# shaderko/velocity-asr

Hardware: NVIDIA B200
Metric: rtfx (higher is better)
Workload: dtype f32

## Files before the change

### velocity-asr_b200/csrc/scan.cu

```cuda
#include <cstdlib>
#include <map>
#include <mutex>
#include <utility>

#include "common.cuh"
#include "kernels.cuh"

namespace vasr {

namespace {

constexpr int SPL = 8;
constexpr int SCAN_THREADS = 128;
constexpr int NLEV = 26;
constexpr float LOG2E = 1.4426950408889634f;

struct State8 {
  u64 v[4];
};

__device__ __forceinline__ void powers_structured(float s, float n0p1, State8& p) {
  const float r1 = ex2_approx(s);
  const float e1 = ex2_approx(s * n0p1);
  const float r2 = r1 * r1;
// ... 477 lines not shown
  float Dv[RPL];
#pragma unroll
  for (int r = 0; r < RPL; ++r) Dv[r] = a.D ? __ldg(a.D + d0 + rl0 + r) : 0.f;

  u64 H[RPL][8];
#pragma unroll
  for (int r = 0; r < RPL; ++r)
#pragma unroll
    for (int k = 0; k < 8; ++k) H[r][k] = 0ull;

  const float* gB = a.Bm + b * L * a.ldb;
  const float* gC = a.Cm + b * L * a.ldc;
  const float* gX = a.x + b * L * a.ldx + d0;
  const float* gDt = a.dt + b * L * a.lddt + d0;
  const float* gZ = gate ? a.z + b * L * a.ldz + d0 : nullptr;
  float* gY = a.y + b * L * a.ldy + d0 + rl0;

  auto issue = [&](int c) {
    const int st = c % 3;
    const int64_t tc0 = (int64_t)c * TCH;
    const int tcn = c >= nchunks ? 0 : (int)((L - tc0) < TCH ? (L - tc0) : TCH);
    float* dB = sB(st); float* dC = sC(st); float* dX = sX(st); float* dD = sDt(st); float* dZ = sZ(st);
#pragma unroll
    for (int i = 0; i < (TCH * NF + THREADS - 1) / THREADS; ++i) {
      const int idx = tid + i * THREADS;
      const int t = idx / NF, f = idx % NF;
      if (idx < TCH * NF && t < tcn) {
        cp_async16(dB + t * N + 4 * f, gB + (tc0 + t) * a.ldb + 4 * f);
        cp_async16(dC + t * N + 4 * f, gC + (tc0 + t) * a.ldc + 4 * f);
      }
    }
#pragma unroll
    for (int i = 0; i < (TCH * RF + THREADS - 1) / THREADS; ++i) {
      const int idx = tid + i * THREADS;
      const int t = idx / RF, f = idx % RF;
      if (idx < TCH * RF && t < tcn) {
        cp_async16(dX + t * ROWS + 4 * f, gX + (tc0 + t) * a.ldx + 4 * f);
        cp_async16(dD + t * ROWS + 4 * f, gDt + (tc0 + t) * a.lddt + 4 * f);
        if (gate) cp_async16(dZ + t * ROWS + 4 * f, gZ + (tc0 + t) * a.ldz + 4 * f);
      }
    }
    cp_async_commit();
  };

  auto row_step = [&](u64 (&Hr)[8], float dtv, float xv, const ulonglong2 (&bq)[4], const ulonglong2 (&cq)[4]) {
    const float u = xv * dtv;
    const u64 uu = pack2(u, u);
    u64 Pa, Pb, rq2 = 0ull;
    if (STRUCT) {
      const float r = ex2_approx(dtv * c_r);
      const float e = ex2_approx(dtv * c_e);
      const float rq = ex2_approx(dtv * c_q);
      const float r2 = r * r;
      Pa = pack2(e, e * r);
      Pb = mul2(Pa, pack2(r2, r2));
      rq2 = pack2(rq, rq);
    }
    u64 acc0 = 0ull, acc1 = 0ull;
#pragma unroll
    for (int m = 0; m < 4; ++m) {
      if (!STRUCT) {
        Pa = pack2(ex2_approx(dtv * al2[4 * m]), ex2_approx(dtv * al2[4 * m + 1]));
        Pb = pack2(ex2_approx(dtv * al2[4 * m + 2]), ex2_approx(dtv * al2[4 * m + 3]));
      }
      Hr[2 * m] = fma2(Pa, Hr[2 * m], mul2(uu, bq[m].x));
      Hr[2 * m + 1] = fma2(Pb, Hr[2 * m + 1], mul2(uu, bq[m].y));
      if (m == 0) {
        acc0 = mul2(Hr[0], cq[0].x);
        acc1 = mul2(Hr[1], cq[0].y);
      } else {
        acc0 = fma2(Hr[2 * m], cq[m].x, acc0);
        acc1 = fma2(Hr[2 * m + 1], cq[m].y, acc1);
      }
      if (STRUCT && m < 3) {
        Pa = mul2(Pa, rq2);
        Pb = mul2(Pb, rq2);
      }
    }
    return hsum2(add2(acc0, acc1));
  };

  struct Pre {
    u64 Pa[RPL], Pb[RPL], rq2[RPL];
    float s[RPL];
  };
  auto row_step_pre = [&](u64 (&Hr)[8], u64 Pa, u64 Pb, u64 rq2, float sc, const ulonglong2 (&bq)[4],
                          const ulonglong2 (&cq)[4]) {
    u64 acc0 = 0ull, acc1 = 0ull;
#pragma unroll
    for (int m = 0; m < 4; ++m) {
      Hr[2 * m] = fma2(Pa, Hr[2 * m], bq[m].x);
      Hr[2 * m + 1] = fma2(Pb, Hr[2 * m + 1], bq[m].y);
      if (m == 0) {
        acc0 = mul2(Hr[0], cq[0].x);
        acc1 = mul2(Hr[1], cq[0].y);
      } else {
        acc0 = fma2(Hr[2 * m], cq[m].x, acc0);
        acc1 = fma2(Hr[2 * m + 1], cq[m].y, acc1);
      }
      if (m < 3) {
        Pa = mul2(Pa, rq2);
        Pb = mul2(Pb, rq2);
      }
    }
    return sc * hsum2(add2(acc0, acc1));
  };
  float s_carry[RPL];
#pragma unroll
  for (int q = 0; q < RPL; ++q) s_carry[q] = 1.0f;

  struct Ops {
    ulonglong2 bq[4], cq[4];
    float dt[RPL], x[RPL];
  };
  auto load_ops = [&](Ops& o, const float* pB, const float* pC, const float* pX, const float* pD, int t) {
#pragma unroll
    for (int m = 0; m < 4; ++m) {
      o.bq[m] = *reinterpret_cast<const ulonglong2*>(pB + t * N + 4 * LPR * m);
      o.cq[m] = *reinterpret_cast<const ulonglong2*>(pC + t * N + 4 * LPR * m);
    }
    if (RPL == 2) {
      const float2 d2 = *reinterpret_cast<const float2*>(pD + t * ROWS);
      const float2 x2 = *reinterpret_cast<const float2*>(pX + t * ROWS);
      o.dt[0] = d2.x; o.dt[RPL - 1] = d2.y; o.x[0] = x2.x; o.x[RPL - 1] = x2.y;
    } else {
#pragma unroll
      for (int r = 0; r < RPL; ++r) { o.dt[r] = pD[t * ROWS + r]; o.x[r] = pX[t * ROWS + r]; }
    }
  };

  constexpr int SPB = TPL / RPL;
  float ypv[NV], fx[TPL], fz[TPL];
#pragma unroll
  for (int i = 0; i < NV; ++i) ypv[i] = 0.f;
#pragma unroll
  for (int i = 0; i < TPL; ++i) fx[i] = fz[i] = 0.f;
  float* fy = gY;
  int fvalid = 0;
  auto finalize = [&]() {
#pragma unroll
    for (int r = 0; r < NR; ++r) {
      const int lane_bit = LPR >> (r + 1);
      const int cnt = (NV / 2) >> r;
      const bool hi = (j & lane_bit) != 0;
#pragma unroll
      for (int i = 0; i < cnt; ++i) {
        const float mine = hi ? ypv[i + cnt] : ypv[i];
        const float other = hi ? ypv[i] : ypv[i + cnt];
        ypv[i] = mine + __shfl_xor_sync(0xffffffffu, other, lane_bit);
      }
    }
#pragma unroll
    for (int sp = 0; sp < SPB; ++sp) {
      float y[RPL];
#pragma unroll
      for (int r = 0; r < RPL; ++r) {
        y[r] = fmaf(fx[sp * RPL + r], Dv[r], ypv[sp * RPL + r]);
        if (gate) {
          const float zv = fz[sp * RPL + r];
          float sg;
          asm("rcp.approx.ftz.f32 %0, %1;" : "=f"(sg) : "f"(1.0f + ex2_approx(-zv * LOG2E)));
          y[r] *= zv * sg;
        }
      }
      if (sp < fvalid) {
        if (RPL == 2) {
          *reinterpret_cast<float2*>(fy + sp * a.ldy) = make_float2(y[0], y[RPL - 1]);
        } else {
#pragma unroll
          for (int r = 0; r < RPL; ++r) fy[sp * a.ldy + r] = y[r];
        }
      }
    }
  };

  constexpr int NST = 3;
  issue(0);
  issue(1);
  for (int c = 0; c < nchunks; ++c) {
    const int st = c % NST;
    const int64_t tc0 = (int64_t)c * TCH;
    const int tcn = (int)((L - tc0) < TCH ? (L - tc0) : TCH);
    cp_async_wait<1>();
    __syncthreads();
    issue(c + 2);
    const float* pB = sB(st) + 4 * j;
    const float* pC = sC(st) + 4 * j;
    const float* pX = sX(st) + rl0;
    const float* pD = sDt(st) + rl0;
    const float* pZ = sZ(st) + rl0;

    Ops cur;
    load_ops(cur, pB, pC, pX, pD, 0);
    Pre pre;
    auto mufu_phase = [&](const Ops& o, float (&r)[RPL], float (&e)[RPL], float (&rq)[RPL]) {
#pragma unroll
      for (int q = 0; q < RPL; ++q) {
        r[q] = ex2_approx(o.dt[q] * c_r);
        e[q] = ex2_approx(o.dt[q] * c_e);
        rq[q] = ex2_approx(o.dt[q] * c_q);
      }
    };
    auto pack_phase = [&](const Ops& o, const float (&r)[RPL], const float (&e)[RPL], const float (&rq)[RPL],
                          const float (&s_prev)[RPL], Pre& p) {
#pragma unroll
      for (int q = 0; q < RPL; ++q) {
        float u = o.x[q] * o.dt[q];
        if (fabsf(u) < 1e-12f) u = copysignf(1e-12f, u);
        float inv;
        asm("rcp.approx.ftz.f32 %0, %1;" : "=f"(inv) : "f"(u));
        const float er = e[q] * (s_prev[q] * inv);
        const float r2 = r[q] * r[q];
        p.Pa[q] = pack2(er, er * r[q]);
        p.Pb[q] = mul2(p.Pa[q], pack2(r2, r2));
        p.rq2[q] = pack2(rq[q], rq[q]);
        p.s[q] = u;
      }
    };
    if (STRUCT) {
      float r[RPL], e[RPL], rq[RPL];
      mufu_phase(cur, r, e, rq);
      pack_phase(cur, r, e, rq, s_carry, pre);
    }
#pragma unroll 4
    for (int g4 = 0; g4 < TCH; g4 += 4) {
      if (g4 >= tcn) break;
      float yp[NV];
#pragma unroll
      for (int i = 0; i < 4; ++i) {
        const int t = g4 + i;
        Ops nxt;
        load_ops(nxt, pB, pC, pX, pD, t + 1 < TCH ? t + 1 : TCH - 1);
        if (STRUCT) {
          float r[RPL], e[RPL], rq[RPL];
          Pre npre;
          yp[RPL * i] = row_step_pre(H[0], pre.Pa[0], pre.Pb[0], pre.rq2[0], pre.s[0], cur.bq, cur.cq);
          mufu_phase(nxt, r, e, rq);
#pragma unroll
          for (int q = 1; q < RPL; ++q)
            yp[RPL * i + q] = row_step_pre(H[q], pre.Pa[q], pre.Pb[q], pre.rq2[q], pre.s[q], cur.bq, cur.cq);
#pragma unroll
          for (int q = 0; q < RPL; ++q) s_carry[q] = pre.s[q];
          pack_phase(nxt, r, e, rq, s_carry, npre);
          pre = npre;
        } else {
#pragma unroll
          for (int r = 0; r < RPL; ++r) yp[RPL * i + r] = row_step(H[r], cur.dt[r], cur.x[r], cur.bq, cur.cq);
        }
        cur = nxt;
      }
      float nfx[TPL], nfz[TPL];
      const int s0 = g4 + j * SPB;
#pragma unroll
      for (int sp = 0; sp < SPB; ++sp) {
        if (RPL == 2) {
          const float2 x2 = *reinterpret_cast<const float2*>(pX + (s0 + sp) * ROWS);
          const float2 z2 = gate ? *reinterpret_cast<const float2*>(pZ + (s0 + sp) * ROWS) : make_float2(0.f, 0.f);
          nfx[sp * RPL] = x2.x; nfx[sp * RPL + RPL - 1] = x2.y;
          nfz[sp * RPL] = z2.x; nfz[sp * RPL + RPL - 1] = z2.y;
        } else {
#pragma unroll
          for (int r = 0; r < RPL; ++r) {
            nfx[sp * RPL + r] = pX[(s0 + sp) * ROWS + r];
            nfz[sp * RPL + r] = gate ? pZ[(s0 + sp) * ROWS + r] : 0.f;
          }
        }
      }
      finalize();
#pragma unroll
      for (int i = 0; i < NV; ++i) ypv[i] = yp[i];
#pragma unroll
      for (int i = 0; i < TPL; ++i) { fx[i] = nfx[i]; fz[i] = nfz[i]; }
      fy = gY + (tc0 + s0) * a.ldy;
      fvalid = tcn - s0;
    }
  }
  pdl_trigger();
  finalize();
}

struct SplitArgs {
  u64* state = nullptr;
  unsigned int* flags = nullptr;
  unsigned int epoch = 0;
  int n_slots = 0;
};

__device__ __forceinline__ u64 shfl_xor2(u64 v, int m) { return __shfl_xor_sync(0xffffffffu, v, m); }
__device__ __forceinline__ u64 bcast2(float v) { return pack2(v, v); }
__device__ __forceinline__ float rcp_approx(float x) {
  float y;
  asm("rcp.approx.ftz.f32 %0, %1;" : "=f"(y) : "f"(x));
  return y;
}
__device__ __forceinline__ unsigned long long global_ns() {
  unsigned long long t;
  asm volatile("mov.u64 %0, %%globaltimer;" : "=l"(t));
  return t;
}

template <int RP, int WARPS, int OCC>
__global__ void __launch_bounds__(WARPS * 32, OCC) scan_rp_kernel(ScanArgs a, SplitArgs sa) {
  pdl_wait();
  constexpr int N = 64, G = 8, R = 2 * RP;
  constexpr int ROWS = WARPS * G * R;
  constexpr int THREADS = WARPS * 32;
  constexpr int LDR = ROWS + 8;
  constexpr int NF = N / 4, RF = ROWS / 4;
  constexpr int STAGE_FLOATS = TCH * (2 * N + 3 * LDR);
  constexpr int NST = 3;
  constexpr int NV = 4 * RP;
  constexpr int SW = RP * 17;

  extern __shared__ __align__(16) float scan_smem[];
  auto sB = [&](int st) { return scan_smem + st * STAGE_FLOATS; };
  auto sC = [&](int st) { return scan_smem + st * STAGE_FLOATS + TCH * N; };
  auto sX = [&](int st) { return scan_smem + st * STAGE_FLOATS + 2 * TCH * N; };
  auto sDt = [&](int st) { return scan_smem + st * STAGE_FLOATS + 2 * TCH * N + TCH * LDR; };
  auto sZ = [&](int st) { return scan_smem + st * STAGE_FLOATS + 2 * TCH * N + 2 * TCH * LDR; };

  const int tid = threadIdx.x;
  const int lane = tid & 31, warp = tid >> 5;
  const int g = lane >> 2, j = lane & 3;
  const int rl0 = (warp * G + g) * R;
  const int64_t L = a.L;
  const bool gate = a.z != nullptr;
  const int tiles = a.Di / ROWS;
  const int64_t cpc = (L + TCH - 1) / TCH;
  const int64_t n_chains = a.B * tiles;

  int64_t f0, f1;
  if (sa.n_slots > 0) {
    const int64_t total = n_chains * cpc;
    f0 = total * blockIdx.x / sa.n_slots;
    f1 = total * (blockIdx.x + 1) / sa.n_slots;
  } else {
    f0 = (int64_t)blockIdx.x * cpc;
    f1 = f0 + cpc;
  }
  if (f1 <= f0) {
    pdl_trigger();
    return;
  }
  const int64_t c_first = f0 / cpc, c_last = (f1 - 1) / cpc;

  const u64 CR = bcast2(-LOG2E);
  const u64 CE = bcast2(-LOG2E * (float)(4 * j + 1));
  const u64 CQ = bcast2(-LOG2E * 16.0f);

  for (int64_t chain = c_last; chain >= c_first; --chain) {
    const int cb = (int)((f0 > chain * cpc ? f0 : chain * cpc) - chain * cpc);
    const int ce = (int)((f1 < (chain + 1) * cpc ? f1 : (chain + 1) * cpc) - chain * cpc);
    const bool load_state = cb > 0, save_state = ce < cpc;
    const bool last_piece = chain == c_first;
    const int64_t b = chain / tiles;
    const int d0 = (int)(chain % tiles) * ROWS;

    u64 DV[RP];
#pragma unroll
    for (int p = 0; p < RP; ++p)
      DV[p] = a.D ? pack2(__ldg(a.D + d0 + rl0 + 2 * p), __ldg(a.D + d0 + rl0 + 2 * p + 1)) : 0ull;

    const float* gB = a.Bm + b * L * a.ldb;
    const float* gC = a.Cm + b * L * a.ldc;
    const float* gX = a.x + b * L * a.ldx + d0;
    const float* gDt = a.dt + b * L * a.lddt + d0;
    const float* gZ = gate ? a.z + b * L * a.ldz + d0 : nullptr;
    float* gY = a.y + b * L * a.ldy + d0 + rl0;

    constexpr int TSB = THREADS / NF, TSX = THREADS / RF;
    static_assert(THREADS % NF == 0 && THREADS % RF == 0 && TCH % TSB == 0 && TCH % TSX == 0, "tile shape");
    const int tb = tid / NF, fb = tid % NF, tx = tid / RF, fx = tid % RF;
    const float* qB = gB + ((int64_t)cb * TCH + tb) * a.ldb + 4 * fb;
    const float* qC = gC + ((int64_t)cb * TCH + tb) * a.ldc + 4 * fb;
    const float* qX = gX + ((int64_t)cb * TCH + tx) * a.ldx + 4 * fx;
    const float* qD = gDt + ((int64_t)cb * TCH + tx) * a.lddt + 4 * fx;
    const float* qZ = gate ? gZ + ((int64_t)cb * TCH + tx) * a.ldz + 4 * fx : nullptr;
    const int oB = tb * N + 4 * fb, oX = tx * LDR + 4 * fx;
    int c_issue = cb;
    auto issue = [&]() {
      const int c = c_issue++;
      if (c < ce) {
        const int st = (c - cb) % NST;
        float* dB = sB(st) + oB; float* dC = sC(st) + oB;
        float* dX = sX(st) + oX; float* dD = sDt(st) + oX; float* dZ = sZ(st) + oX;
        const int64_t left = L - (int64_t)c * TCH;
        if (left >= TCH) {
#pragma unroll
          for (int i = 0; i < TCH / TSB; ++i) {
            cp_async16(dB + i * TSB * N, qB + (int64_t)i * TSB * a.ldb);
            cp_async16(dC + i * TSB * N, qC + (int64_t)i * TSB * a.ldc);
          }
#pragma unroll
          for (int i = 0; i < TCH / TSX; ++i) {
            cp_async16(dX + i * TSX * LDR, qX + (int64_t)i * TSX * a.ldx);
            cp_async16(dD + i * TSX * LDR, qD + (int64_t)i * TSX * a.lddt);
            if (gate) cp_async16(dZ + i * TSX * LDR, qZ + (int64_t)i * TSX * a.ldz);
          }
        } else {
#pragma unroll
          for (int i = 0; i < TCH / TSB; ++i)
            if (tb + i * TSB < left) {
              cp_async16(dB + i * TSB * N, qB + (int64_t)i * TSB * a.ldb);
              cp_async16(dC + i * TSB * N, qC + (int64_t)i * TSB * a.ldc);
            }
#pragma unroll
          for (int i = 0; i < TCH / TSX; ++i)
            if (tx + i * TSX < left) {
              cp_async16(dX + i * TSX * LDR, qX + (int64_t)i * TSX * a.ldx);
              cp_async16(dD + i * TSX * LDR, qD + (int64_t)i * TSX * a.lddt);
              if (gate) cp_async16(dZ + i * TSX * LDR, qZ + (int64_t)i * TSX * a.ldz);
            }
        }
        qB += (int64_t)TCH * a.ldb; qC += (int64_t)TCH * a.ldc;
        qX += (int64_t)TCH * a.ldx; qD += (int64_t)TCH * a.lddt;
        if (gate) qZ += (int64_t)TCH * a.ldz;
      }
      cp_async_commit();
    };
#pragma unroll
    for (int i = 0; i < NST - 1; ++i) issue();

    u64 H[RP][16];
    u64 s_carry[RP];
    if (load_state) {
      if (tid == 0) {
        const volatile unsigned int* fl = sa.flags + (blockIdx.x - 1);
        const unsigned long long t0 = global_ns();
        while (*fl != sa.epoch) {
          __nanosleep(100);
          if (global_ns() - t0 > 4000000000ull) __trap();
        }
        __threadfence();
      }
      __syncthreads();
      const u64* st = sa.state + (size_t)(blockIdx.x - 1) * THREADS * SW + tid;
#pragma unroll
      for (int p = 0; p < RP; ++p) {
#pragma unroll
        for (int k = 0; k < 16; ++k) H[p][k] = __ldcg(st + (size_t)(p * 16 + k) * THREADS);
        s_carry[p] = __ldcg(st + (size_t)(RP * 16 + p) * THREADS);
      }
    } else {
#pragma unroll
      for (int p = 0; p < RP; ++p) {
#pragma unroll
        for (int k = 0; k < 16; ++k) H[p][k] = 0ull;
        s_carry[p] = bcast2(1.0f);
      }
    }

    struct Pre {
      u64 ER[RP], R1[RP], R2[RP], RQ[RP], S[RP];
    };
    struct Raw {
      float r[R], e[R], q[R], u[R], inv[R];
    };
    auto load_dx = [&](u64 (&DT)[RP], u64 (&X)[RP], const float* pD, const float* pX, int t) {
      if (RP == 2) {
        const ulonglong2 d = *reinterpret_cast<const ulonglong2*>(pD + t * LDR);
        const ulonglong2 x = *reinterpret_cast<const ulonglong2*>(pX + t * LDR);
        DT[0] = d.x; DT[RP - 1] = d.y; X[0] = x.x; X[RP - 1] = x.y;
      } else {
        DT[0] = *reinterpret_cast<const u64*>(pD + t * LDR);
        X[0] = *reinterpret_cast<const u64*>(pX + t * LDR);
      }
    };
    auto mufu_phase = [&](const u64 (&DT)[RP], const u64 (&X)[RP], Raw& w) {
#pragma unroll
      for (int p = 0; p < RP; ++p) {
        float a0, a1;
        unpack2(mul2(DT[p], CR), a0, a1);
        w.r[2 * p] = ex2_approx(a0); w.r[2 * p + 1] = ex2_approx(a1);
        unpack2(mul2(DT[p], CE), a0, a1);
        w.e[2 * p] = ex2_approx(a0); w.e[2 * p + 1] = ex2_approx(a1);
        unpack2(mul2(DT[p], CQ), a0, a1);
        w.q[2 * p] = ex2_approx(a0); w.q[2 * p + 1] = ex2_approx(a1);
        unpack2(mul2(X[p], DT[p]), a0, a1);
        if (fabsf(a0) < 1e-12f) a0 = copysignf(1e-12f, a0);
        if (fabsf(a1) < 1e-12f) a1 = copysignf(1e-12f, a1);
        w.u[2 * p] = a0; w.u[2 * p + 1] = a1;
        w.inv[2 * p] = rcp_approx(a0); w.inv[2 * p + 1] = rcp_approx(a1);
      }
    };
    auto pack_phase = [&](const Raw& w, const u64 (&s_prev)[RP], Pre& o) {
#pragma unroll
      for (int p = 0; p < RP; ++p) {
        const u64 ratio = mul2(s_prev[p], pack2(w.inv[2 * p], w.inv[2 * p + 1]));
        o.ER[p] = mul2(pack2(w.e[2 * p], w.e[2 * p + 1]), ratio);
        o.R1[p] = pack2(w.r[2 * p], w.r[2 * p + 1]);
        o.R2[p] = mul2(o.R1[p], o.R1[p]);
        o.RQ[p] = pack2(w.q[2 * p], w.q[2 * p + 1]);
        o.S[p] = pack2(w.u[2 * p], w.u[2 * p + 1]);
      }
    };

    u64 ypv[NV], FX[RP], FZ[RP];
#pragma unroll
    for (int i = 0; i < NV; ++i) ypv[i] = 0ull;
#pragma unroll
    for (int p = 0; p < RP; ++p) FX[p] = FZ[p] = 0ull;
    float* fy = gY;
    bool fvalid = false;
    auto finalize = [&]() {
#pragma unroll
      for (int r = 0; r < 2; ++r) {
        const int lane_bit = 2 >> r;
        const int cnt = (NV / 2) >> r;
        const bool hi = (j & lane_bit) != 0;
#pragma unroll
        for (int i = 0; i < cnt; ++i) {
          const u64 mine = hi ? ypv[i + cnt] : ypv[i];
          const u64 other = hi ? ypv[i] : ypv[i + cnt];
          ypv[i] = add2(mine, shfl_xor2(other, lane_bit));
        }
      }
      float out[R];
#pragma unroll
      for (int p = 0; p < RP; ++p) {
        u64 y = fma2(FX[p], DV[p], ypv[p]);
        if (gate) {
          float e0, e1;
          unpack2(mul2(FZ[p], CR), e0, e1);
          const u64 sg = pack2(rcp_approx(1.0f + ex2_approx(e0)), rcp_approx(1.0f + ex2_approx(e1)));
          y = mul2(y, mul2(FZ[p], sg));
        }
        unpack2(y, out[2 * p], out[2 * p + 1]);
      }
      if (fvalid) {
        if (RP == 2) *reinterpret_cast<float4*>(fy) = make_float4(out[0], out[1], out[R - 2], out[R - 1]);
        else *reinterpret_cast<float2*>(fy) = make_float2(out[0], out[1]);
      }
    };

    cp_async_wait<NST - 2>();
    __syncthreads();
    Pre pre;
    {
      u64 DT[RP], X[RP];
      Raw w;
      load_dx(DT, X, sDt(0) + rl0, sX(0) + rl0, 0);
      mufu_phase(DT, X, w);
      pack_phase(w, s_carry, pre);
    }
    for (int c = cb; c < ce; ++c) {
      const int st = (c - cb) % NST, stn = (c + 1 - cb) % NST;
      const int64_t tc0 = (int64_t)c * TCH;
      const int tcn = (int)((L - tc0) < TCH ? (L - tc0) : TCH);
      if (last_piece && c + 1 == ce) pdl_trigger();
      const float* pB = sB(st) + 4 * j;
      const float* pC = sC(st) + 4 * j;
      const float* pX = sX(st) + rl0;
      const float* pD = sDt(st) + rl0;
      const float* pZ = sZ(st) + rl0;
#pragma unroll 1
      for (int g4 = 0; g4 < TCH; g4 += 4) {
        if (g4 >= tcn) break;
        const bool last_block = g4 + 4 == TCH;
        if (last_block) {
          cp_async_wait<0>();
          __syncthreads();
          issue();
        }
        const float* pDl = last_block ? sDt(stn) + rl0 : pD + (g4 + 4) * LDR;
        const float* pXl = last_block ? sX(stn) + rl0 : pX + (g4 + 4) * LDR;
        u64 yp[NV];
#pragma unroll
        for (int i = 0; i < 4; ++i) {
          const int t = g4 + i;
          u64 DTn[RP], Xn[RP];
          Raw w;
          Pre npre;
          if (i < 3) load_dx(DTn, Xn, pD, pX, t + 1);
          else load_dx(DTn, Xn, pDl, pXl, 0);
          u64 P[RP][4], acc[RP][2];
#pragma unroll
          for (int p = 0; p < RP; ++p) {
            P[p][0] = pre.ER[p];
            P[p][1] = mul2(pre.ER[p], pre.R1[p]);
            P[p][2] = mul2(pre.ER[p], pre.R2[p]);
            P[p][3] = mul2(P[p][1], pre.R2[p]);
          }
#pragma unroll
          for (int m = 0; m < 4; ++m) {
            const float4 bq = *reinterpret_cast<const float4*>(pB + t * N + 16 * m);
            const float4 cq = *reinterpret_cast<const float4*>(pC + t * N + 16 * m);
            const float bv[4] = {bq.x, bq.y, bq.z, bq.w};
            const float cv[4] = {cq.x, cq.y, cq.z, cq.w};
#pragma unroll
            for (int p = 0; p < RP; ++p) {
#pragma unroll
              for (int q = 0; q < 4; ++q) {
                u64& h = H[p][4 * m + q];
                h = fma2(P[p][q], h, bcast2(bv[q]));
                if (m == 0 && q < 2) acc[p][q] = mul2(h, bcast2(cv[q]));
                else acc[p][q & 1] = fma2(h, bcast2(cv[q]), acc[p][q & 1]);
                if (m < 3) P[p][q] = mul2(P[p][q], pre.RQ[p]);
              }
            }
            if (m == 0) mufu_phase(DTn, Xn, w);
          }
#pragma unroll
          for (int p = 0; p < RP; ++p) {
            yp[RP * i + p] = mul2(add2(acc[p][0], acc[p][1]), pre.S[p]);
            s_carry[p] = pre.S[p];
          }
          pack_phase(w, s_carry, npre);
          pre = npre;
        }
        u64 nFX[RP], nFZ[RP];
        const int s0 = g4 + j;
        if (RP == 2) {
          const ulonglong2 x2 = *reinterpret_cast<const ulonglong2*>(pX + s0 * LDR);
          nFX[0] = x2.x; nFX[RP - 1] = x2.y;
          if (gate) {
            const ulonglong2 z2 = *reinterpret_cast<const ulonglong2*>(pZ + s0 * LDR);
            nFZ[0] = z2.x; nFZ[RP - 1] = z2.y;
          } else {
            nFZ[0] = nFZ[RP - 1] = 0ull;
          }
        } else {
          nFX[0] = *reinterpret_cast<const u64*>(pX + s0 * LDR);
          nFZ[0] = gate ? *reinterpret_cast<const u64*>(pZ + s0 * LDR) : 0ull;
        }
        finalize();
#pragma unroll
        for (int i = 0; i < NV; ++i) ypv[i] = yp[i];
#pragma unroll
        for (int p = 0; p < RP; ++p) { FX[p] = nFX[p]; FZ[p] = nFZ[p]; }
        fy = gY + (tc0 + s0) * a.ldy;
        fvalid = s0 < tcn;
      }
    }
    finalize();
    cp_async_wait<0>();

    if (save_state) {
      u64* st = sa.state + (size_t)blockIdx.x * THREADS * SW + tid;
#pragma unroll
      for (int p = 0; p < RP; ++p) {
#pragma unroll
        for (int k = 0; k < 16; ++k) __stcg(st + (size_t)(p * 16 + k) * THREADS, H[p][k]);
        __stcg(st + (size_t)(RP * 16 + p) * THREADS, s_carry[p]);
      }
      __threadfence();
      __syncthreads();
      if (tid == 0) *reinterpret_cast<volatile unsigned int*>(sa.flags + blockIdx.x) = sa.epoch;
    } else {
      __syncthreads();
    }
  }
}

constexpr int RP_WARPS = 4;
template <int RP, int OCC = 3>
struct RpCfg {
  static constexpr int ROWS = RP_WARPS * 8 * 2 * RP;
  static constexpr int THREADS = RP_WARPS * 32;
  static constexpr size_t SMEM = (size_t)3 * TCH * (2 * 64 + 3 * (ROWS + 8)) * sizeof(float);
  static constexpr size_t STATE_BYTES = (size_t)THREADS * RP * 17 * sizeof(unsigned long long);
};
constexpr int RP_MAX_SLOTS = 1024;
constexpr size_t RP_SCRATCH_BYTES = 4096 + (size_t)RP_MAX_SLOTS * RpCfg<2>::STATE_BYTES;

struct RpScratch {
  void* mem = nullptr;
  unsigned int epoch = 0;
};
cudaError_t rp_scratch(cudaStream_t s, RpScratch** out) {
  static std::mutex mu;
  static std::map<std::pair<int, cudaStream_t>, RpScratch> cache;
  int dev = 0;
  cudaError_t e = cudaGetDevice(&dev);
  if (e != cudaSuccess) return e;
  std::lock_guard<std::mutex> lock(mu);
  RpScratch& sc = cache[std::make_pair(dev, s)];
  if (!sc.mem) {
    e = cudaMalloc(&sc.mem, RP_SCRATCH_BYTES);
    if (e != cudaSuccess) return e;
    e = cudaMemset(sc.mem, 0, 4096);
    if (e != cudaSuccess) return e;
  }
  *out = &sc;
  return cudaSuccess;
}

bool rp_takes(const ScanArgs& a) {
  auto al16 = [](const void* p) { return (reinterpret_cast<uintptr_t>(p) & 15) == 0; };
  if (a.parallel_quirk || !a.structured_a || a.N != 64 || a.Di % RpCfg<1>::ROWS != 0) return false;
  if ((a.ldx & 3) || (a.lddt & 3) || (a.ldy & 3) || (a.ldb & 3) || (a.ldc & 3)) return false;
  if (!al16(a.x) || !al16(a.dt) || !al16(a.y) || !al16(a.Bm) || !al16(a.Cm)) return false;
  if (a.z && ((a.ldz & 3) || !al16(a.z))) return false;
  return true;
}

template <int RP, int OCC>
cudaError_t launch_rp_cfg(const ScanArgs& a, int sms, cudaStream_t s) {
  using C = RpCfg<RP, OCC>;
  auto kernel = scan_rp_kernel<RP, RP_WARPS, OCC>;
  constexpr size_t SPLIT_SMEM = C::SMEM > 78 * 1024 ? C::SMEM : 78 * 1024;
  static int occ = -1;
  cudaError_t e = cudaSuccess;
  if (occ < 0) {
    e = cudaFuncSetAttribute(kernel, cudaFuncAttributeMaxDynamicSharedMemorySize, (int)SPLIT_SMEM);
    if (e != cudaSuccess) return e;
    int n = 0;
    e = cudaOccupancyMaxActiveBlocksPerMultiprocessor(&n, kernel, C::THREADS, C::SMEM);
    if (e != cudaSuccess) return e;
    occ = n;
  }
  const int64_t n_chains = a.B * (a.Di / C::ROWS);
  const int64_t total = n_chains * ((a.L + TCH - 1) / TCH);
  SplitArgs sa;
  unsigned grid = (unsigned)n_chains;
  size_t smem = C::SMEM;
  int64_t slots = (int64_t)(occ < 2 ? occ : 2) * sms;
  if (slots > RP_MAX_SLOTS) slots = RP_MAX_SLOTS;
  if (slots > total) slots = total;
  static const int split_env = debug_env_int("VASR_SCAN_SPLIT", -1);
  if (split_env > 0 && split_env <= (int64_t)occ * sms && split_env <= RP_MAX_SLOTS) slots = split_env;
  bool split = occ > 0 && n_chains > slots && slots >= 1 && n_chains % slots != 0;
  if (split_env == 0) split = false;
  if (split) {
    RpScratch* sc = nullptr;
    e = rp_scratch(s, &sc);
    if (e != cudaSuccess) return e;
    sa.n_slots = (int)slots;
    sa.flags = reinterpret_cast<unsigned int*>(sc->mem);
    sa.state = reinterpret_cast<u64*>(reinterpret_cast<char*>(sc->mem) + 4096);
    if (++sc->epoch == 0) ++sc->epoch;
    sa.epoch = sc->epoch;
    grid = (unsigned)slots;
    smem = SPLIT_SMEM;
  }
  return launch_k(kernel, dim3(grid), dim3(C::THREADS), smem, s, a, sa);
}

cudaError_t launch_rp(const ScanArgs& a, cudaStream_t s) {
  const int sms = a.num_sms > 0 ? a.num_sms : 148;
  static const int rp_env = debug_env_int("VASR_SCAN_RP", 0);
  const bool wide = rp_env ? rp_env == 2 : a.B * (a.Di / RpCfg<2>::ROWS) >= 2 * sms;
  if (a.Di % RpCfg<2>::ROWS == 0 && wide) {
    return launch_rp_cfg<2, 2>(a, sms, s);
  }
  return launch_rp_cfg<1, 3>(a, sms, s);
}

template <int LPR, int WARPS, int RPL>
cudaError_t launch_seq(const ScanArgs& a, cudaStream_t s) {
  constexpr int N = LPR * 16;
  constexpr int ROWS = WARPS * (32 / LPR) * RPL;
  constexpr size_t SMEM = (size_t)3 * TCH * (2 * N + 3 * ROWS) * sizeof(float);
  dim3 grid((unsigned)(a.Di / ROWS), (unsigned)a.B);
  cudaError_t e = cudaSuccess;
  auto go = [&](auto kernel) {
    if (SMEM > 48 * 1024) e = cudaFuncSetAttribute(kernel, cudaFuncAttributeMaxDynamicSharedMemorySize, (int)SMEM);
    if (e == cudaSuccess) e = launch_k(kernel, grid, dim3(WARPS * 32), SMEM, s, a);
  };
  if (a.structured_a) go(scan_seq_kernel<LPR, WARPS, RPL, true>);
  else go(scan_seq_kernel<LPR, WARPS, RPL, false>);
  return e;
}

template <int LPR>
cudaError_t launch_recurrence(const ScanArgs& a, cudaStream_t s) {
  constexpr int G = 32 / LPR;
  auto al16 = [](const void* p) { return (reinterpret_cast<uintptr_t>(p) & 15) == 0; };
  if ((a.ldx & 3) || (a.lddt & 3) || (a.ldy & 1) || !al16(a.x) || !al16(a.dt) || (a.z && ((a.ldz & 3) || !al16(a.z))) ||
      (reinterpret_cast<uintptr_t>(a.y) & 7))
    return cudaErrorInvalidValue;
  if (4 * G * 2 <= 128 && a.Di % (4 * G * 2) == 0) return launch_seq<LPR, 4, 2>(a, s);
  if (2 * G * 2 <= 128 && a.Di % (2 * G * 2) == 0) return launch_seq<LPR, 2, 2>(a, s);
  if (a.Di % (G * 2) == 0) return launch_seq<LPR, 1, 2>(a, s);
  return cudaErrorInvalidValue;
}

template <int LPR8>
cudaError_t launch_lpr(const ScanArgs& a, cudaStream_t s) {
  if (!a.parallel_quirk) return launch_recurrence<LPR8 / 2>(a, s);
  constexpr int ROWS = SCAN_THREADS / LPR8;
  if (a.Di % ROWS != 0) return cudaErrorInvalidValue;
  dim3 grid((unsigned)(a.Di / ROWS), (unsigned)a.B);
  if (a.structured_a) return launch_k(scan_quirk_kernel<LPR8, true>, grid, dim3(SCAN_THREADS), 0, s, a);
  return launch_k(scan_quirk_kernel<LPR8, false>, grid, dim3(SCAN_THREADS), 0, s, a);
}

}

cudaError_t launch_selective_scan(const ScanArgs& a, cudaStream_t s, int64_t* launches) {
  if (a.B <= 0 || a.L <= 0) return cudaSuccess;
  if (a.B > 65535 || a.L >= (1LL << (NLEV - 2))) return cudaErrorInvalidValue;
  if ((a.ldb & 3) || (a.ldc & 3) || (reinterpret_cast<uintptr_t>(a.Bm) & 15) ||
      (reinterpret_cast<uintptr_t>(a.Cm) & 15))
    return cudaErrorInvalidValue;
  cudaError_t e;
  static const int old_env = debug_env_int("VASR_SCAN_OLD", 0);
  if (rp_takes(a) && !old_env) {
    e = launch_rp(a, s);
    if (launches && e == cudaSuccess) ++*launches;
    return e;
  }
  switch (a.N) {
    case 64: e = launch_lpr<8>(a, s); break;
    case 32: e = launch_lpr<4>(a, s); break;
    case 16: e = launch_lpr<2>(a, s); break;
    default: return cudaErrorInvalidValue;
  }
  if (launches && e == cudaSuccess) ++*launches;
  return e;
}

}
```

Baseline: 192,000.

## Precompute per-row scan seeds in shared memory and halve state per lane

Adds a per-chunk prep pass that computes decay exponentials, the ratio of consecutive u values and u itself once per row, storing them in a double-buffered shared seed area. The main loop then loads these instead of redoing the MUFU exp and reciprocal work per lane. Lanes are regrouped to 8 per row group, so each lane carries 8 state pairs instead of 16, and the s_carry rescaling moves into finalize. The RP=1 path is dropped. This adds shared memory and a prep step inside the pipeline, and the extra smem may lower occupancy.

```diff
diff --git a/velocity-asr_b200/csrc/scan.cu b/velocity-asr_b200/csrc/scan.cu
--- a/velocity-asr_b200/csrc/scan.cu
+++ b/velocity-asr_b200/csrc/scan.cu
@@ -803,7 +803,8 @@
 template <int RP, int WARPS, int OCC>
 __global__ void __launch_bounds__(WARPS * 32, OCC) scan_rp_kernel(ScanArgs a, SplitArgs sa) {
   pdl_wait();
-  constexpr int N = 64, G = 8, R = 2 * RP;
+  static_assert(RP == 2, "row pairs per lane: the seed pre-pass covers a warp's rows with two lanes per row");
+  constexpr int N = 64, G = 4, R = 2 * RP;
   constexpr int ROWS = WARPS * G * R;
   constexpr int THREADS = WARPS * 32;
   constexpr int LDR = ROWS + 8;
@@ -811,7 +812,10 @@
   constexpr int STAGE_FLOATS = TCH * (2 * N + 3 * LDR);
   constexpr int NST = 3;
   constexpr int NV = 4 * RP;
-  constexpr int SW = RP * 17;
+  constexpr int FP = RP / 2;
+  constexpr int SW = RP * 8;
+  constexpr int WR = G * R;
+  static_assert(32 % WR == 0 && 32 / WR == 2, "prep: two lanes per row, half a chunk each");
 
   extern __shared__ __align__(16) float scan_smem[];
   auto sB = [&](int st) { return scan_smem + st * STAGE_FLOATS; };
@@ -819,11 +823,13 @@
   auto sX = [&](int st) { return scan_smem + st * STAGE_FLOATS + 2 * TCH * N; };
   auto sDt = [&](int st) { return scan_smem + st * STAGE_FLOATS + 2 * TCH * N + TCH * LDR; };
   auto sZ = [&](int st) { return scan_smem + st * STAGE_FLOATS + 2 * TCH * N + 2 * TCH * LDR; };
+  auto sSeed = [&](int buf) { return scan_smem + NST * STAGE_FLOATS + buf * 4 * TCH * ROWS; };
 
   const int tid = threadIdx.x;
   const int lane = tid & 31, warp = tid >> 5;
-  const int g = lane >> 2, j = lane & 3;
+  const int g = lane >> 3, j = lane & 7;
   const int rl0 = (warp * G + g) * R;
+  const int rf0 = rl0 + 2 * FP * (j & 1);
   const int64_t L = a.L;
   const bool gate = a.z != nullptr;
   const int tiles = a.Di / ROWS;
@@ -847,7 +853,6 @@
 
   const u64 CR = bcast2(-LOG2E);
   const u64 CE = bcast2(-LOG2E * (float)(4 * j + 1));
-  const u64 CQ = bcast2(-LOG2E * 16.0f);
 
   for (int64_t chain = c_last; chain >= c_first; --chain) {
     const int cb = (int)((f0 > chain * cpc ? f0 : chain * cpc) - chain * cpc);
@@ -857,17 +862,17 @@
     const int64_t b = chain / tiles;
     const int d0 = (int)(chain % tiles) * ROWS;
 
-    u64 DV[RP];
-#pragma unroll
-    for (int p = 0; p < RP; ++p)
-      DV[p] = a.D ? pack2(__ldg(a.D + d0 + rl0 + 2 * p), __ldg(a.D + d0 + rl0 + 2 * p + 1)) : 0ull;
+    u64 DV[FP];
+#pragma unroll
+    for (int p = 0; p < FP; ++p)
+      DV[p] = a.D ? pack2(__ldg(a.D + d0 + rf0 + 2 * p), __ldg(a.D + d0 + rf0 + 2 * p + 1)) : 0ull;
 
     const float* gB = a.Bm + b * L * a.ldb;
     const float* gC = a.Cm + b * L * a.ldc;
     const float* gX = a.x + b * L * a.ldx + d0;
     const float* gDt = a.dt + b * L * a.lddt + d0;
     const float* gZ = gate ? a.z + b * L * a.ldz + d0 : nullptr;
-    float* gY = a.y + b * L * a.ldy + d0 + rl0;
+    float* gY = a.y + b * L * a.ldy + d0 + rf0;
 
     constexpr int TSB = THREADS / NF, TSX = THREADS / RF;
     static_assert(THREADS % NF == 0 && THREADS % RF == 0 && TCH % TSB == 0 && TCH % TSX == 0, "tile shape");
@@ -922,8 +927,7 @@
 #pragma unroll
     for (int i = 0; i < NST - 1; ++i) issue();
 
-    u64 H[RP][16];
-    u64 s_carry[RP];
+    u64 H[RP][8];
     if (load_state) {
       if (tid == 0) {
         const volatile unsigned int* fl = sa.flags + (blockIdx.x - 1);
@@ -937,76 +941,78 @@
       __syncthreads();
       const u64* st = sa.state + (size_t)(blockIdx.x - 1) * THREADS * SW + tid;
 #pragma unroll
-      for (int p = 0; p < RP; ++p) {
-#pragma unroll
-        for (int k = 0; k < 16; ++k) H[p][k] = __ldcg(st + (size_t)(p * 16 + k) * THREADS);
-        s_carry[p] = __ldcg(st + (size_t)(RP * 16 + p) * THREADS);
-      }
+      for (int p = 0; p < RP; ++p)
+#pragma unroll
+        for (int k = 0; k < 8; ++k) H[p][k] = __ldcg(st + (size_t)(p * 8 + k) * THREADS);
     } else {
 #pragma unroll
-      for (int p = 0; p < RP; ++p) {
-#pragma unroll
-        for (int k = 0; k < 16; ++k) H[p][k] = 0ull;
-        s_carry[p] = bcast2(1.0f);
-      }
-    }
-
-    struct Pre {
-      u64 ER[RP], R1[RP], R2[RP], RQ[RP], S[RP];
+      for (int p = 0; p < RP; ++p)
+#pragma unroll
+        for (int k = 0; k < 8; ++k) H[p][k] = 0ull;
+    }
+
+    auto clampu = [](float u) { return fabsf(u) < 1e-12f ? copysignf(1e-12f, u) : u; };
+    auto prep = [&](int c, int st_c, int st_p, int buf) {
+      const int r = warp * WR + (lane % WR);
+      const int t0 = (lane / WR) * (TCH / 2);
+      const float* X = sX(st_c) + r;
+      const float* D = sDt(st_c) + r;
+      float up;
+      if (t0 > 0) up = clampu(X[(t0 - 1) * LDR] * D[(t0 - 1) * LDR]);
+      else if (c > cb) up = clampu(sX(st_p)[(TCH - 1) * LDR + r] * sDt(st_p)[(TCH - 1) * LDR + r]);
+      else if (c > 0) up = clampu(__ldg(gX + ((int64_t)c * TCH - 1) * a.ldx + r) * __ldg(gDt + ((int64_t)c * TCH - 1) * a.lddt + r));
+      else up = 1.0f;
+      float* o = sSeed(buf) + r;
+#pragma unroll
+      for (int k = 0; k < TCH / 2; ++k) {
+        const int t = t0 + k;
+        const float dtv = D[t * LDR];
+        const float u = clampu(X[t * LDR] * dtv);
+        o[(0 * TCH + t) * ROWS] = ex2_approx(dtv * -LOG2E);
+        o[(1 * TCH + t) * ROWS] = ex2_approx(dtv * (-LOG2E * 32.0f));
+        o[(2 * TCH + t) * ROWS] = up * rcp_approx(u);
+        o[(3 * TCH + t) * ROWS] = u;
+        up = u;
+      }
+      __syncwarp();
     };
-    struct Raw {
-      float r[R], e[R], q[R], u[R], inv[R];
+
+    struct Ops {
+      u64 DT[RP], R1[RP], RQ[RP], RT[RP];
     };
-    auto load_dx = [&](u64 (&DT)[RP], u64 (&X)[RP], const float* pD, const float* pX, int t) {
-      if (RP == 2) {
-        const ulonglong2 d = *reinterpret_cast<const ulonglong2*>(pD + t * LDR);
-        const ulonglong2 x = *reinterpret_cast<const ulonglong2*>(pX + t * LDR);
-        DT[0] = d.x; DT[RP - 1] = d.y; X[0] = x.x; X[RP - 1] = x.y;
-      } else {
-        DT[0] = *reinterpret_cast<const u64*>(pD + t * LDR);
-        X[0] = *reinterpret_cast<const u64*>(pX + t * LDR);
+    auto load_ops = [&](Ops& o, const float* pD, const float* pS, int t) {
+#pragma unroll
+      for (int h = 0; h < RP / 2; ++h) {
+        const ulonglong2 d = *reinterpret_cast<const ulonglong2*>(pD + t * LDR + 4 * h);
+        const ulonglong2 r1 = *reinterpret_cast<const ulonglong2*>(pS + (0 * TCH + t) * ROWS + 4 * h);
+        const ulonglong2 rq = *reinterpret_cast<const ulonglong2*>(pS + (1 * TCH + t) * ROWS + 4 * h);
+        const ulonglong2 rt = *reinterpret_cast<const ulonglong2*>(pS + (2 * TCH + t) * ROWS + 4 * h);
+        o.DT[2 * h] = d.x; o.DT[2 * h + 1] = d.y;
+        o.R1[2 * h] = r1.x; o.R1[2 * h + 1] = r1.y;
+        o.RQ[2 * h] = rq.x; o.RQ[2 * h + 1] = rq.y;
+        o.RT[2 * h] = rt.x; o.RT[2 * h + 1] = rt.y;
       }
     };
-    auto mufu_phase = [&](const u64 (&DT)[RP], const u64 (&X)[RP], Raw& w) {
+    auto mufu_phase = [&](const Ops& o, float (&e)[R]) {
 #pragma unroll
       for (int p = 0; p < RP; ++p) {
         float a0, a1;
-        unpack2(mul2(DT[p], CR), a0, a1);
-        w.r[2 * p] = ex2_approx(a0); w.r[2 * p + 1] = ex2_approx(a1);
-        unpack2(mul2(DT[p], CE), a0, a1);
-        w.e[2 * p] = ex2_approx(a0); w.e[2 * p + 1] = ex2_approx(a1);
-        unpack2(mul2(DT[p], CQ), a0, a1);
-        w.q[2 * p] = ex2_approx(a0); w.q[2 * p + 1] = ex2_approx(a1);
-        unpack2(mul2(X[p], DT[p]), a0, a1);
-        if (fabsf(a0) < 1e-12f) a0 = copysignf(1e-12f, a0);
-        if (fabsf(a1) < 1e-12f) a1 = copysignf(1e-12f, a1);
-        w.u[2 * p] = a0; w.u[2 * p + 1] = a1;
-        w.inv[2 * p] = rcp_approx(a0); w.inv[2 * p + 1] = rcp_approx(a1);
+        unpack2(mul2(o.DT[p], CE), a0, a1);
+        e[2 * p] = ex2_approx(a0); e[2 * p + 1] = ex2_approx(a1);
       }
     };
-    auto pack_phase = [&](const Raw& w, const u64 (&s_prev)[RP], Pre& o) {
-#pragma unroll
-      for (int p = 0; p < RP; ++p) {
-        const u64 ratio = mul2(s_prev[p], pack2(w.inv[2 * p], w.inv[2 * p + 1]));
-        o.ER[p] = mul2(pack2(w.e[2 * p], w.e[2 * p + 1]), ratio);
-        o.R1[p] = pack2(w.r[2 * p], w.r[2 * p + 1]);
-        o.R2[p] = mul2(o.R1[p], o.R1[p]);
-        o.RQ[p] = pack2(w.q[2 * p], w.q[2 * p + 1]);
-        o.S[p] = pack2(w.u[2 * p], w.u[2 * p + 1]);
-      }
-    };
-
-    u64 ypv[NV], FX[RP], FZ[RP];
+
+    u64 ypv[NV], FX[FP], FZ[FP], FS[FP];
 #pragma unroll
     for (int i = 0; i < NV; ++i) ypv[i] = 0ull;
 #pragma unroll
-    for (int p = 0; p < RP; ++p) FX[p] = FZ[p] = 0ull;
+    for (int p = 0; p < FP; ++p) FX[p] = FZ[p] = FS[p] = 0ull;
     float* fy = gY;
     bool fvalid = false;
     auto finalize = [&]() {
 #pragma unroll
-      for (int r = 0; r < 2; ++r) {
-        const int lane_bit = 2 >> r;
+      for (int r = 0; r < 3; ++r) {
+        const int lane_bit = 4 >> r;
         const int cnt = (NV / 2) >> r;
         const bool hi = (j & lane_bit) != 0;
 #pragma unroll
@@ -1016,10 +1022,10 @@
           ypv[i] = add2(mine, shfl_xor2(other, lane_bit));
         }
       }
-      float out[R];
-#pragma unroll
-      for (int p = 0; p < RP; ++p) {
-        u64 y = fma2(FX[p], DV[p], ypv[p]);
+      float out[2 * FP];
+#pragma unroll
+      for (int p = 0; p < FP; ++p) {
+        u64 y = fma2(FX[p], DV[p], mul2(ypv[p], FS[p]));
         if (gate) {
           float e0, e1;
           unpack2(mul2(FZ[p], CR), e0, e1);
@@ -1029,31 +1035,31 @@
         unpack2(y, out[2 * p], out[2 * p + 1]);
       }
       if (fvalid) {
-        if (RP == 2) *reinterpret_cast<float4*>(fy) = make_float4(out[0], out[1], out[R - 2], out[R - 1]);
+        if (FP == 2) *reinterpret_cast<float4*>(fy) = make_float4(out[0], out[1], out[2 * FP - 2], out[2 * FP - 1]);
         else *reinterpret_cast<float2*>(fy) = make_float2(out[0], out[1]);
       }
     };
 
     cp_async_wait<NST - 2>();
     __syncthreads();
-    Pre pre;
-    {
-      u64 DT[RP], X[RP];
-      Raw w;
-      load_dx(DT, X, sDt(0) + rl0, sX(0) + rl0, 0);
-      mufu_phase(DT, X, w);
-      pack_phase(w, s_carry, pre);
-    }
+    prep(cb, 0, 0, 0);
+    Ops cur;
+    float ecur[R];
+    load_ops(cur, sDt(0) + rl0, sSeed(0) + rl0, 0);
+    mufu_phase(cur, ecur);
     for (int c = cb; c < ce; ++c) {
       const int st = (c - cb) % NST, stn = (c + 1 - cb) % NST;
+      const int sb = (c - cb) & 1;
       const int64_t tc0 = (int64_t)c * TCH;
       const int tcn = (int)((L - tc0) < TCH ? (L - tc0) : TCH);
       if (last_piece && c + 1 == ce) pdl_trigger();
       const float* pB = sB(st) + 4 * j;
       const float* pC = sC(st) + 4 * j;
-      const float* pX = sX(st) + rl0;
       const float* pD = sDt(st) + rl0;
-      const float* pZ = sZ(st) + rl0;
+      const float* pS = sSeed(sb) + rl0;
+      const float* pXf = sX(st) + rf0;
+      const float* pZf = sZ(st) + rf0;
+      const float* pSf = sSeed(sb) + 3 * TCH * ROWS + rf0;
 #pragma unroll 1
       for (int g4 = 0; g4 < TCH; g4 += 4) {
         if (g4 >= tcn) break;
@@ -1062,30 +1068,30 @@
           cp_async_wait<0>();
           __syncthreads();
           issue();
+          if (c + 1 < ce) prep(c + 1, stn, st, sb ^ 1);
         }
         const float* pDl = last_block ? sDt(stn) + rl0 : pD + (g4 + 4) * LDR;
-        const float* pXl = last_block ? sX(stn) + rl0 : pX + (g4 + 4) * LDR;
+        const float* pSl = last_block ? sSeed(sb ^ 1) + rl0 : pS + (g4 + 4) * ROWS;
         u64 yp[NV];
 #pragma unroll
         for (int i = 0; i < 4; ++i) {
           const int t = g4 + i;
-          u64 DTn[RP], Xn[RP];
-          Raw w;
-          Pre npre;
-          if (i < 3) load_dx(DTn, Xn, pD, pX, t + 1);
-          else load_dx(DTn, Xn, pDl, pXl, 0);
-          u64 P[RP][4], acc[RP][2];
+          Ops nxt;
+          float enxt[R];
+          if (i < 3) load_ops(nxt, pD, pS, t + 1);
+          else load_ops(nxt, pDl, pSl, 0);
+          u64 P[RP][4], acc[RP];
 #pragma unroll
           for (int p = 0; p < RP; ++p) {
-            P[p][0] = pre.ER[p];
-            P[p][1] = mul2(pre.ER[p], pre.R1[p]);
-            P[p][2] = mul2(pre.ER[p], pre.R2[p]);
-            P[p][3] = mul2(P[p][1], pre.R2[p]);
+            P[p][0] = mul2(pack2(ecur[2 * p], ecur[2 * p + 1]), cur.RT[p]);
+            P[p][1] = mul2(P[p][0], cur.R1[p]);
+            P[p][2] = mul2(P[p][1], cur.R1[p]);
+            P[p][3] = mul2(P[p][2], cur.R1[p]);
           }
 #pragma unroll
-          for (int m = 0; m < 4; ++m) {
-            const float4 bq = *reinterpret_cast<const float4*>(pB + t * N + 16 * m);
-            const float4 cq = *reinterpret_cast<const float4*>(pC + t * N + 16 * m);
+          for (int m = 0; m < 2; ++m) {
+            const float4 bq = *reinterpret_cast<const float4*>(pB + t * N + 32 * m);
+            const float4 cq = *reinterpret_cast<const float4*>(pC + t * N + 32 * m);
             const float bv[4] = {bq.x, bq.y, bq.z, bq.w};
             const float cv[4] = {cq.x, cq.y, cq.z, cq.w};
 #pragma unroll
@@ -1094,41 +1100,41 @@
               for (int q = 0; q < 4; ++q) {
                 u64& h = H[p][4 * m + q];
                 h = fma2(P[p][q], h, bcast2(bv[q]));
-                if (m == 0 && q < 2) acc[p][q] = mul2(h, bcast2(cv[q]));
-                else acc[p][q & 1] = fma2(h, bcast2(cv[q]), acc[p][q & 1]);
-                if (m < 3) P[p][q] = mul2(P[p][q], pre.RQ[p]);
+                acc[p] = (m == 0 && q == 0) ? mul2(h, bcast2(cv[q])) : fma2(h, bcast2(cv[q]), acc[p]);
+                if (m == 0) P[p][q] = mul2(P[p][q], cur.RQ[p]);
               }
             }
-            if (m == 0) mufu_phase(DTn, Xn, w);
+            if (m == 0) mufu_phase(nxt, enxt);
           }
 #pragma unroll
-          for (int p = 0; p < RP; ++p) {
-            yp[RP * i + p] = mul2(add2(acc[p][0], acc[p][1]), pre.S[p]);
-            s_carry[p] = pre.S[p];
-          }
-          pack_phase(w, s_carry, npre);
-          pre = npre;
-        }
-        u64 nFX[RP], nFZ[RP];
-        const int s0 = g4 + j;
-        if (RP == 2) {
-          const ulonglong2 x2 = *reinterpret_cast<const ulonglong2*>(pX + s0 * LDR);
-          nFX[0] = x2.x; nFX[RP - 1] = x2.y;
+          for (int p = 0; p < RP; ++p) yp[RP * i + p] = acc[p];
+          cur = nxt;
+#pragma unroll
+          for (int k = 0; k < R; ++k) ecur[k] = enxt[k];
+        }
+        u64 nFX[FP], nFZ[FP], nFS[FP];
+        const int s0 = g4 + (j >> 1);
+        if (FP == 2) {
+          const ulonglong2 x2 = *reinterpret_cast<const ulonglong2*>(pXf + s0 * LDR);
+          const ulonglong2 u2 = *reinterpret_cast<const ulonglong2*>(pSf + s0 * ROWS);
+          nFX[0] = x2.x; nFX[FP - 1] = x2.y;
+          nFS[0] = u2.x; nFS[FP - 1] = u2.y;
           if (gate) {
-            const ulonglong2 z2 = *reinterpret_cast<const ulonglong2*>(pZ + s0 * LDR);
-            nFZ[0] = z2.x; nFZ[RP - 1] = z2.y;
+            const ulonglong2 z2 = *reinterpret_cast<const ulonglong2*>(pZf + s0 * LDR);
+            nFZ[0] = z2.x; nFZ[FP - 1] = z2.y;
           } else {
-            nFZ[0] = nFZ[RP - 1] = 0ull;
+            nFZ[0] = nFZ[FP - 1] = 0ull;
           }
         } else {
-          nFX[0] = *reinterpret_cast<const u64*>(pX + s0 * LDR);
-          nFZ[0] = gate ? *reinterpret_cast<const u64*>(pZ + s0 * LDR) : 0ull;
+          nFX[0] = *reinterpret_cast<const u64*>(pXf + s0 * LDR);
+          nFS[0] = *reinterpret_cast<const u64*>(pSf + s0 * ROWS);
+          nFZ[0] = gate ? *reinterpret_cast<const u64*>(pZf + s0 * LDR) : 0ull;
         }
         finalize();
 #pragma unroll
         for (int i = 0; i < NV; ++i) ypv[i] = yp[i];
 #pragma unroll
-        for (int p = 0; p < RP; ++p) { FX[p] = nFX[p]; FZ[p] = nFZ[p]; }
+        for (int p = 0; p < FP; ++p) { FX[p] = nFX[p]; FZ[p] = nFZ[p]; FS[p] = nFS[p]; }
         fy = gY + (tc0 + s0) * a.ldy;
         fvalid = s0 < tcn;
       }
@@ -1139,11 +1145,9 @@
     if (save_state) {
       u64* st = sa.state + (size_t)blockIdx.x * THREADS * SW + tid;
 #pragma unroll
-      for (int p = 0; p < RP; ++p) {
-#pragma unroll
-        for (int k = 0; k < 16; ++k) __stcg(st + (size_t)(p * 16 + k) * THREADS, H[p][k]);
-        __stcg(st + (size_t)(RP * 16 + p) * THREADS, s_carry[p]);
-      }
+      for (int p = 0; p < RP; ++p)
+#pragma unroll
+        for (int k = 0; k < 8; ++k) __stcg(st + (size_t)(p * 8 + k) * THREADS, H[p][k]);
       __threadfence();
       __syncthreads();
       if (tid == 0) *reinterpret_cast<volatile unsigned int*>(sa.flags + blockIdx.x) = sa.epoch;
@@ -1154,12 +1158,12 @@
 }
 
 constexpr int RP_WARPS = 4;
-template <int RP, int OCC = 3>
+template <int RP, int OCC = 2>
 struct RpCfg {
-  static constexpr int ROWS = RP_WARPS * 8 * 2 * RP;
+  static constexpr int ROWS = RP_WARPS * 4 * 2 * RP;
   static constexpr int THREADS = RP_WARPS * 32;
-  static constexpr size_t SMEM = (size_t)3 * TCH * (2 * 64 + 3 * (ROWS + 8)) * sizeof(float);
-  static constexpr size_t STATE_BYTES = (size_t)THREADS * RP * 17 * sizeof(unsigned long long);
+  static constexpr size_t SMEM = ((size_t)3 * TCH * (2 * 64 + 3 * (ROWS + 8)) + (size_t)2 * 4 * TCH * ROWS) * sizeof(float);
+  static constexpr size_t STATE_BYTES = (size_t)THREADS * RP * 8 * sizeof(unsigned long long);
 };
 constexpr int RP_MAX_SLOTS = 1024;
 constexpr size_t RP_SCRATCH_BYTES = 4096 + (size_t)RP_MAX_SLOTS * RpCfg<2>::STATE_BYTES;
@@ -1188,7 +1192,7 @@
 
 bool rp_takes(const ScanArgs& a) {
   auto al16 = [](const void* p) { return (reinterpret_cast<uintptr_t>(p) & 15) == 0; };
-  if (a.parallel_quirk || !a.structured_a || a.N != 64 || a.Di % RpCfg<1>::ROWS != 0) return false;
+  if (a.parallel_quirk || !a.structured_a || a.N != 64 || a.Di % RpCfg<2>::ROWS != 0) return false;
   if ((a.ldx & 3) || (a.lddt & 3) || (a.ldy & 3) || (a.ldb & 3) || (a.ldc & 3)) return false;
   if (!al16(a.x) || !al16(a.dt) || !al16(a.y) || !al16(a.Bm) || !al16(a.Cm)) return false;
   if (a.z && ((a.ldz & 3) || !al16(a.z))) return false;
@@ -1232,19 +1236,13 @@
     if (++sc->epoch == 0) ++sc->epoch;
     sa.epoch = sc->epoch;
     grid = (unsigned)slots;
-    smem = SPLIT_SMEM;
+    smem = slots > 2 * (int64_t)sms ? C::SMEM : SPLIT_SMEM;
   }
   return launch_k(kernel, dim3(grid), dim3(C::THREADS), smem, s, a, sa);
 }
 
 cudaError_t launch_rp(const ScanArgs& a, cudaStream_t s) {
-  const int sms = a.num_sms > 0 ? a.num_sms : 148;
-  static const int rp_env = debug_env_int("VASR_SCAN_RP", 0);
-  const bool wide = rp_env ? rp_env == 2 : a.B * (a.Di / RpCfg<2>::ROWS) >= 2 * sms;
-  if (a.Di % RpCfg<2>::ROWS == 0 && wide) {
-    return launch_rp_cfg<2, 2>(a, sms, s);
-  }
-  return launch_rp_cfg<1, 3>(a, sms, s);
+  return launch_rp_cfg<2, 2>(a, a.num_sms > 0 ? a.num_sms : 148, s);
 }
 
 template <int LPR, int WARPS, int RPL>
```

Result: slower. 189,200 (median of 6 runs) (-1.5%).
